# isri-aist/NMPC

Hardware: AMD Instinct MI355X
Metric: DDP iterations/s (whole node), batch=4096, T=100 (higher is better)
Workload: dtype f64

## Files before the change

### include/nmpc_amd/hip/ddp_kernels_quad.hpp

```cpp
#pragma once

#include <type_traits>

#include <nmpc_amd/hip/ddp_kernels_2w.hpp>

namespace nmpc_amd
{
namespace hip
{
constexpr int kQuadInstances = 16;
constexpr int kQuadWaves = 4;

template<class Problem, bool kConstrained, bool kFanOut = kConstrained>
struct QuadSolver : PairSolver<Problem, kConstrained, true, (kConstrained || kFanOut) ? 4 : 1, true>
{
  using Pair = PairSolver<Problem, kConstrained, true, (kConstrained || kFanOut) ? 4 : 1, true>;
  using Base = typename Pair::Base;
  using Base::b;
  using Base::buf;
  using Base::cfg;
  using Base::current_t;
  using Base::dV0;
  using Base::dV1;
  using Base::k_rel_norm;
  using Base::lambda;
  using Base::lane;
  using Base::problem;
  using Base::sel;
  using Base::T;
  static constexpr int N = Base::N;
  static constexpr int M = Base::M;
  static constexpr int MM = Base::MM;
  static constexpr size_t LW = Base::LW;
  using typename Base::InputDimVector;
  using typename Base::InputInputDimMatrix;
  using typename Base::QPOut;
  using typename Base::StateDimVector;
  using typename Base::StateInputDimMatrix;
  using typename Base::StateStateDimMatrix;

  static constexpr bool kShape = (N >= 1 && N <= 4 && M == 1 && !Problem::kDynamicInput);

  static constexpr int oFx = 0;
  static constexpr int oLxx = 16;
  static constexpr int oFu = 32;
  static constexpr int oLxu = 36;
  static constexpr int oLx = 40;
  static constexpr int oLuu = 44;
  static constexpr int oLu = 45;
  static constexpr int oU = 46;
  static constexpr int oLoRel = 46;
  static constexpr int oUpRel = 48;
  static constexpr int oZero = 47;
  static constexpr int kRecQ = 49;
  static constexpr int kChunkSteps = 16;
  static constexpr int gK = 0;
  static constexpr int gKfb = 1;
  static constexpr int gLive = 5;
  static constexpr int gDummy = 6;
  static constexpr int kGainRec = 7;
  static constexpr int kInstPad = 8;
  static constexpr int kChunkDoubles = 64 * (kRecQ + kGainRec) + 4 * kInstPad;
  static constexpr int kMailIn = 4;
  static constexpr int kMailOut = 4;
  static constexpr int kMailDoubles = (kMailIn + kMailOut) * kQuadInstances;
  static constexpr int kLdsDoubles = Pair::kLdsDoubles + kMailDoubles + kQuadWaves * kChunkDoubles;
  static constexpr size_t kLdsBytes = static_cast<size_t>(kLdsDoubles) * sizeof(double);

  const Problem & lin_problem;
  const int wave;
  const int wl;
  const int row, blk, col;
  double * mail;
  double * chunk;

  NMPC_D QuadSolver(const Problem & p,
                    const Problem & p_lin,
                    const nmpc_hip_ddp_config & c,
                    const DeviceBuffers & bf,
                    int global_lane,
                    double * lds_base)
  : Pair(p, c, bf, global_lane, lds_base), lin_problem(p_lin), wave(threadIdx.x / 64), wl(threadIdx.x % 64), row(wl / 16), blk((wl / 4) % 4),
    col(wl % 4), mail(lds_base + Pair::kLdsDoubles),
    chunk(lds_base + Pair::kLdsDoubles + kMailDoubles + (threadIdx.x / 64) * kChunkDoubles)
  {
  }

  NMPC_D double & mailIn(int inst, int f) const
  {
    return mail[f * kQuadInstances + inst];
  }
  NMPC_D double & mailOut(int inst, int f) const
  {
    return mail[(kMailIn + f) * kQuadInstances + inst];
  }

  NMPC_D static double mma(double a, double b_, double c)
  {
    return __builtin_amdgcn_mfma_f64_4x4x4f64(a, b_, c, 0, 0, 0);
  }
  template<int kSrc>
  NMPC_D static double quadBroadcast(double v)
  {
    constexpr int ctrl = kSrc | (kSrc << 2) | (kSrc << 4) | (kSrc << 6);
    const int lo = __builtin_amdgcn_update_dpp(0, __double2loint(v), ctrl, 0xf, 0xf, true);
    const int hi = __builtin_amdgcn_update_dpp(0, __double2hiint(v), ctrl, 0xf, 0xf, true);
    return __hiloint2double(hi, lo);
  }
  NMPC_D static double pick(bool p, double v)
  {
    return p ? v : 0.0;
  }

  struct PointQ
  {
    double x[N], u;
    double lo, hi;
  };
  NMPC_D static void loadPointQ(int i, const double * px, const double * pu, PointQ & p)
  {
#pragma unroll
    for(int j = 0; j < N; j++)
    {
      p.x[j] = px[(static_cast<size_t>(i) * N + j) * LW];
    }
    p.u = pu[static_cast<size_t>(i) * LW];
  }
  template<bool kFull>
  NMPC_D static void put(double * at, double v)
  {
    if(kFull || !__builtin_constant_p(v))
    {
      *at = v;
    }
  }
  template<bool kFull>
  NMPC_D double lineariseStep(int i, double t0_l, const PointQ & p, double * rec) const
  {
    const double t = t0_l + i * lin_problem.dt();
    StateDimVector x;
    InputDimVector u;
    u.resize(M);
#pragma unroll
    for(int j = 0; j < N; j++)
    {
      x[j] = p.x[j];
    }
    u[0] = p.u;
    StateStateDimMatrix Fx, Lxx;
    StateInputDimMatrix Fu, Lxu;
    StateDimVector Lx;
    InputDimVector Lu;
    InputInputDimMatrix Luu;
    Fu.resize(N, M);
    Lxu.resize(N, M);
    Lu.resize(M);
    Luu.resize(M, M);
    lin_problem.calcStateEqDeriv(t, x, u, Fx, Fu);
    lin_problem.calcRunningCostDeriv(t, x, u, Lx, Lu, Lxx, Luu, Lxu);
#pragma unroll
    for(int r = 0; r < 4; r++)
    {
#pragma unroll
      for(int c = 0; c < 4; c++)
      {
        put<kFull>(rec + oFx + 4 * r + c, (r < N && c < N) ? Fx(r < N ? r : 0, c < N ? c : 0) : 0.0);
        put<kFull>(rec + oLxx + 4 * r + c, (r < N && c < N) ? Lxx(r < N ? r : 0, c < N ? c : 0) : 0.0);
      }
      put<kFull>(rec + oFu + r, (r < N) ? Fu(r < N ? r : 0, 0) : 0.0);
      put<kFull>(rec + oLxu + r, (r < N) ? Lxu(r < N ? r : 0, 0) : 0.0);
      put<kFull>(rec + oLx + r, (r < N) ? Lx[r < N ? r : 0] : 0.0);
    }
    put<kFull>(rec + oLuu, Luu(0, 0));
    put<kFull>(rec + oLu, Lu[0]);
    if constexpr(kConstrained)
    {
      rec[oLoRel] = p.lo - u[0];
      rec[oUpRel] = p.hi - u[0];
    }
    else
    {
      rec[oU] = u[0];
    }
    put<kFull>(rec + oZero, 0.0);
    return recipFast(fabs(u[0]) + 1.0);
  }

  NMPC_D void backwardQuad() const
  {
    const int inst = wave * 4 + blk;
    const bool need = mailIn(inst, 0) != 0.0;
    const double lam = mailIn(inst, 1);
    const int lane_q = static_cast<int>(lane - lane % kQuadInstances) + inst;
    const int inst_l = wave * 4 + wl / 16;
    const int ts_l = wl % 16;
    const int sel_l = static_cast<int>(mailIn(inst_l, 2));
    const double t0_l = mailIn(inst_l, 3);
    const int lane_l = static_cast<int>(lane - lane % kQuadInstances) + inst_l;
    const double * px = Base::Xt + static_cast<size_t>(sel_l) * (Base::rowsX() * LW) + lane_l;
    const double * pu = Base::Ut + static_cast<size_t>(sel_l) * (Base::rowsU() * LW) + lane_l;
    double * rec_l = chunk + static_cast<size_t>(wl) * kRecQ + (wl / 16) * kInstPad;
    double * gains = chunk + 64 * kRecQ + 4 * kInstPad;
    const double * gain_l = gains + static_cast<size_t>(wl) * kGainRec;
    double * gain_q = gains + static_cast<size_t>(blk * 16) * kGainRec
                      + (row == 0 ? gKfb + col : ((row == 1 && col == 0) ? gK : ((row == 1 && col == 1) ? gLive : gDummy)));
    double * gain_u = gains + static_cast<size_t>(blk * 16) * kGainRec
                      + (row == 0 ? gKfb + col : ((row == 1 && col == 0) ? gK : gDummy));
    double * live_q = gains + static_cast<size_t>(blk * 16 + 4 * row + col) * kGainRec + gLive;
    const double * rec_q = chunk + static_cast<size_t>(blk * 16) * kRecQ + blk * kInstPad;

    const bool c0 = col == 0, c1 = col == 1, r0 = row == 0;
    const int aE = 4 * row + col;
    const int aT = 4 * col + row;
    const int aFuM = c0 ? oFu + row : oZero;
    const int aFuB = oFu + row;
    const int aLM = c0 ? oLxu + row : (c1 ? oLx + row : oZero);
    const int aCM = c0 ? oLuu : (c1 ? oLu : oZero);
    const int aLxuRow = oLxu + col;
    struct Operands
    {
      double Fx, Lxx, LxxT, FuM, FuB, LM, CM, LxuRow, lo, up;
    };
    auto loadOperands = [&](int ts, Operands & o)
    {
      const double * R = rec_q + static_cast<size_t>(ts) * kRecQ;
      o.Fx = R[oFx + aE];
      o.Lxx = R[oLxx + aE];
      o.LxxT = R[oLxx + aT];
      o.FuM = R[aFuM];
      o.FuB = R[aFuB];
      o.LM = R[aLM];
      o.CM = R[aCM];
      o.LxuRow = R[aLxuRow];
      if constexpr(kConstrained)
      {
        o.lo = R[oLoRel];
        o.up = R[oUpRel];
      }
    };

    if(ts_l == 0)
    {
      StateDimVector xT, vx;
      StateStateDimMatrix vxx;
#pragma unroll
      for(int j = 0; j < N; j++)
      {
        xT[j] = px[(static_cast<size_t>(T) * N + j) * LW];
      }
      lin_problem.calcTerminalCostDeriv(t0_l + T * lin_problem.dt(), xT, vx, vxx);
#pragma unroll
      for(int r = 0; r < 4; r++)
      {
#pragma unroll
        for(int c = 0; c < 4; c++)
        {
          rec_l[4 * r + c] = (r < N && c < N) ? vxx(r < N ? r : 0, c < N ? c : 0) : 0.0;
        }
        rec_l[16 + r] = (r < N) ? vx[r < N ? r : 0] : 0.0;
      }
    }
    double Vxx = rec_q[aE];
    double VxM = pick(c1, rec_q[16 + row]);

    double dV0_l = 0, dV1_l = 0;
    bool ok = true;
    double k_next = 0;
    bool have_next = false;
    const size_t tile_T = static_cast<size_t>(T);
    const int b_q = b - static_cast<int>(lane) + lane_q;

    auto step = [&](auto reg_tag, auto guarded_tag, int i, int ts, const Operands & o, int ts_next, Operands & o_next)
    {
      constexpr int kReg = decltype(reg_tag)::value;
      constexpr bool kGuarded = decltype(guarded_tag)::value;
      loadOperands(ts_next, o_next);
      const double P = mma(Vxx, o.Fx, 0.0);
      const double Rm = mma(Vxx, o.FuM, VxM);
      const double Qxx = mma(P, o.Fx, o.Lxx);
      const double QxxT = mma(o.Fx, P, o.LxxT);
      const double S = mma(o.Fx, Rm, o.LM);
      const double Wq = mma(o.FuB, Rm, o.CM);
      const double QA = mma(quadBroadcast<0>(Rm), o.Fx, o.LxuRow);
      const double Quu = quadBroadcast<0>(Wq);
      const double Qu = quadBroadcast<1>(Wq);
      const double Qr = quadBroadcast<0>(S);
      const double Qxr = quadBroadcast<1>(S);

      double Quu_F = Quu, QAr = QA, Qrr = Qr;
      if constexpr(kReg == 2)
      {
        const double VxxReg = (row == col) ? Vxx + lam : Vxx;
        const double R2 = mma(VxxReg, o.FuM, 0.0);
        Quu_F = quadBroadcast<0>(mma(o.FuB, R2, o.CM));
        QAr = mma(quadBroadcast<0>(R2), o.Fx, o.LxuRow);
        Qrr = quadBroadcast<0>(mma(o.Fx, R2, o.LM));
      }
      else if constexpr(kReg == 1)
      {
        Quu_F = Quu + lam;
      }

      double k, inv;
      bool step_ok;
      [[maybe_unused]] double qp_code = 0;
      if constexpr(kConstrained)
      {
        const double initial_k = (i != T - 1 && have_next) ? k_next : 0.0;
        QPOut qp;
#ifdef NMPC_AMD_PROFILE_QP
        asm volatile("s_nop 0" ::"v"(Quu_F), "v"(Qu));
        const unsigned long long tq = __builtin_readcyclecounter();
#endif
        Base::boxQP1Fast(Quu_F, Qu, o.lo, o.up, initial_k, qp);
#ifdef NMPC_AMD_PROFILE_QP
        asm volatile("s_nop 0" ::"v"(qp.x[0]), "v"(qp.retval));
        Pair::prof_wait += __builtin_readcyclecounter() - tq;
#endif
        qp_code = (need && ok) ? static_cast<double>(4 * (qp.retval + 8) + (qp.n_free > 0 ? 2 : 0)) : 0.0;
        step_ok = qp.retval >= 0;
        k = step_ok ? qp.x[0] : 0.0;
        inv = (step_ok && qp.n_free > 0) ? qp.inv_d[0] : 0.0;
      }
      else
      {
        step_ok = !(Quu_F <= 0);
        inv = (!kGuarded || step_ok) ? recipFast(Quu_F) : 0.0;
        k = -1 * (Qu * inv);
      }
      const double Kc = -1 * (QAr * inv);
      const double Kr = -1 * (Qrr * inv);
      const bool live = need && ok && step_ok;
      ok = ok && step_ok;

      if(!kGuarded || live)
      {
        dV0_l += k * Qu;
        dV1_l += 0.5 * (k * (Quu * k));
      }
      const double KQr = Kr * Quu, KQc = Kc * Quu;
      const double Vn = fma(Qr, Kc, fma(Kr, QA, fma(KQr, Kc, Qxx)));
      const double VnT = fma(QA, Kr, fma(Kc, Qr, fma(KQc, Kr, QxxT)));
      Vxx = 0.5 * (Vn + VnT);
      VxM = pick(c1, fma(Qr, k, fma(Kr, Qu, fma(KQr, k, Qxr))));

      if constexpr(kGuarded)
      {
        gain_q[static_cast<size_t>(ts) * kGainRec] = r0 ? Kc : (c0 ? k : (kConstrained ? qp_code + (live ? 1.0 : 0.0) : (live ? 1.0 : 0.0)));
      }
      else
      {
        gain_u[static_cast<size_t>(ts) * kGainRec] = r0 ? Kc : k;
      }
      k_next = k;
      have_next = true;
    };

    const int b_l = b - static_cast<int>(lane) + lane_l;
    auto loadLimits = [&](int i, PointQ & p)
    {
      if constexpr(kConstrained)
      {
        p.lo = inputLimitLo(buf, b_l, i, 0);
        p.hi = inputLimitHi(buf, b_l, i, 0);
      }
    };
    double krn_l = 0;
    auto flushGains = [&](int i_first, double uinv)
    {
      const int i = i_first + ts_l;
      const double flag = (i < T) ? gain_l[gLive] : 0.0;
      bool save = flag != 0.0;
      if constexpr(kConstrained)
      {
        const int code = static_cast<int>(flag);
        if(save)
        {
          Base::tileBase(buf.qp_ret, tile_T)[static_cast<size_t>(i) * LW + lane_l] = (code >> 2) - 8;
          Base::tileBase(buf.qp_free, tile_T)[static_cast<size_t>(i) * LW + lane_l] = static_cast<unsigned>((code >> 1) & 1);
        }
        save = (code & 1) != 0;
      }
      if(save)
      {
        const double kv = gain_l[gK];
        Base::kt[static_cast<size_t>(i) * LW + lane_l] = kv;
#pragma unroll
        for(int c = 0; c < N; c++)
        {
          Base::Kt[(static_cast<size_t>(i) * N + c) * LW + lane_l] = gain_l[gKfb + c];
        }
        krn_l = fmax(krn_l, fabs(kv) * uinv);
      }
    };
    auto runChunks = [&](auto reg_tag)
    {
      const int n_chunks = (T + kChunkSteps - 1) / kChunkSteps;
      PointQ pt;
      {
        const int i = ((n_chunks - 1) * kChunkSteps + ts_l < T) ? (n_chunks - 1) * kChunkSteps + ts_l : T - 1;
        loadPointQ(i, px, pu, pt);
        loadLimits(i, pt);
      }
      double uinv_prev = 0;
      for(int ch = n_chunks - 1; ch >= 0; ch--)
      {
        const int i0 = ch * kChunkSteps;
        double uinv_now;
        {
#ifdef NMPC_AMD_PROFILE_2W
          const unsigned long long tl = __builtin_readcyclecounter();
#endif
          const int i = (i0 + ts_l < T) ? i0 + ts_l : T - 1;
          uinv_now = (ch == n_chunks - 1) ? lineariseStep<true>(i, t0_l, pt, rec_l) : lineariseStep<false>(i, t0_l, pt, rec_l);
#ifdef NMPC_AMD_PROFILE_2W
          asm volatile("s_waitcnt lgkmcnt(0)" ::: "memory");
#ifndef NMPC_AMD_PROFILE_QP
          Pair::prof_wait += __builtin_readcyclecounter() - tl;
#endif
          Pair::prof_count++;
#endif
        }
        if(ch + 1 < n_chunks)
        {
          flushGains(i0 + kChunkSteps, uinv_prev);
        }
        uinv_prev = uinv_now;
        if(!Pair::kNominalTail || ch > 0)
        {
          const int in = i0 - kChunkSteps + ts_l;
          loadPointQ(in > 0 ? in : 0, px, pu, pt);
          loadLimits(in > 0 ? in : 0, pt);
        }
        const int hi = (i0 + kChunkSteps - 1 < T) ? i0 + kChunkSteps - 1 : T - 1;
#ifdef NMPC_AMD_QUAD_NO_STRAIGHT
        if constexpr(false)
#else
        if constexpr(!kConstrained)
#endif
        {
          const int n_steps = hi - i0 + 1;
          if((n_steps == kChunkSteps || n_steps == 4) && __all(ok))
          {
            const double Vxx_s = Vxx, VxM_s = VxM, dV0_s = dV0_l, dV1_s = dV1_l;
            auto straight = [&](auto r_tag)
            {
              constexpr int R = decltype(r_tag)::value;
              Operands o2[2];
              loadOperands(R - 1, o2[(R - 1) & 1]);
#pragma unroll
              for(int ts = R - 1; ts >= 0; ts--)
              {
                step(reg_tag, std::false_type(), i0 + ts, ts, o2[ts & 1], ts > 0 ? ts - 1 : 0, o2[(ts & 1) ^ 1]);
              }
            };
            if(n_steps == kChunkSteps)
            {
              straight(std::integral_constant<int, kChunkSteps>());
            }
            else
            {
              straight(std::integral_constant<int, 4>());
            }
            if(__all(ok))
            {
              *live_q = need ? 1.0 : 0.0;
              continue;
            }
            Vxx = Vxx_s;
            VxM = VxM_s;
            dV0_l = dV0_s;
            dV1_l = dV1_s;
            ok = true;
          }
        }
        Operands oa, ob;
        loadOperands(hi - i0, oa);
        int i = hi;
        for(; i - 1 >= i0; i -= 2)
        {
          step(reg_tag, std::true_type(), i, i - i0, oa, i - 1 - i0, ob);
          step(reg_tag, std::true_type(), i - 1, i - 1 - i0, ob, (i - 2 >= i0) ? i - 2 - i0 : 0, oa);
        }
        if(i >= i0)
        {
          step(reg_tag, std::true_type(), i, i - i0, oa, 0, ob);
        }
      }
      flushGains(0, uinv_prev);
      if constexpr(Pair::kNominalTail)
      {
        asm volatile("" ::: "memory");
        if(ts_l < 3 * Pair::kFwdGroup)
        {
          double * rec = Pair::nomRec(ts_l / Pair::kFwdGroup, ts_l % Pair::kFwdGroup, static_cast<unsigned>(inst_l));
#pragma unroll
          for(int j = 0; j < N; j++)
          {
            rec[j] = pt.x[j];
          }
          rec[N] = pt.u;
          rec[N + 1] = gain_l[gK];
#pragma unroll
          for(int c = 0; c < N; c++)
          {
            rec[N + 2 + c] = gain_l[gKfb + c];
          }
          if constexpr(Pair::kNomRec > N + 2 + N)
          {
            rec[Pair::kNomRec - 1] = 0;
          }
        }
      }
    };
    if(cfg.reg_type == 2)
    {
      runChunks(std::integral_constant<int, 2>());
    }
    else if(cfg.reg_type == 1)
    {
      runChunks(std::integral_constant<int, 1>());
    }
    else
    {
      runChunks(std::integral_constant<int, 0>());
    }
#pragma unroll
    for(int m = 8; m >= 1; m >>= 1)
    {
      krn_l = fmax(krn_l, __shfl_xor(krn_l, m, 16));
    }
    if(ts_l == 0)
    {
      mailOut(inst_l, 3) = krn_l;
    }
    if(r0 && c0)
    {
      mailOut(inst, 0) = ok ? 1.0 : 0.0;
      mailOut(inst, 1) = dV0_l;
      mailOut(inst, 2) = dV1_l;
    }
    fullBarrier();
  }

  NMPC_D bool backwardMasterQuad(bool need)
  {
    const int inst = wl % kQuadInstances;
    if(wl < kQuadInstances)
    {
      mailIn(inst, 0) = need ? 1.0 : 0.0;
      mailIn(inst, 1) = lambda;
      mailIn(inst, 2) = static_cast<double>(sel);
      mailIn(inst, 3) = current_t;
    }
    Pair::post(Pair::kCmdBackward);
    Pair::profBegin();
    backwardQuad();
    Pair::profEnd(0);
    const bool ok = mailOut(inst, 0) != 0.0;
    if(need)
    {
      dV0 = mailOut(inst, 1);
      dV1 = mailOut(inst, 2);
      k_rel_norm = mailOut(inst, 3);
    }
    return ok;
  }

  template<bool kResumable = false>
  NMPC_D void solveMasterQuad(bool valid)
  {
    if constexpr(kConstrained || kFanOut)
    {
      Pair::template solveMasterFanOut<kResumable>(valid, [this](bool need) { return backwardMasterQuad(need); });
    }
    else
    {
      Pair::template solveMasterWith<kResumable>(valid, [this](bool need) { return backwardMasterQuad(need); });
    }
  }

  NMPC_D void followerLoop() const
  {
    for(;;)
    {
      fullBarrier();
      const int word = static_cast<int>(Pair::mailFlags());
      const int cmd = __builtin_amdgcn_readfirstlane(word >> 1);
      const int sel_h = word & 1;
      if(cmd == Pair::kCmdExit)
      {
#ifdef NMPC_AMD_PROFILE_2W
        if(blockIdx.x == 0 && wl == 0)
        {
          buf.qp_free[static_cast<size_t>(4 + wave) * LW] = __builtin_amdgcn_s_getreg((15 << 11) | (0 << 6) | 4);
        }
#endif
        return;
      }
      if(cmd == Pair::kCmdBackward)
      {
        backwardQuad();
      }
      else if(cmd == Pair::kCmdAdoptFanOut)
      {
        Pair::adoptFanOut(sel_h);
      }
      else if(wave == 1)
      {
        if(cmd == Pair::kCmdForwardFanOut)
        {
          Pair::template forwardHelper<true>(sel_h);
        }
        else
        {
          Pair::forwardHelper(sel_h, cmd == Pair::kCmdRollout);
        }
      }
      else if(Pair::kExtraMasters > 0 && cmd == Pair::kCmdForwardFanOut && Pair::mailWidePass() != 0.0)
      {
        if(wave == 2)
        {
          Pair::template forwardCostOnlyLds<true>(sel_h, 0);
        }
        else
        {
          Pair::template forwardCostOnlyLds<false>(sel_h, 1);
        }
      }
      else if(Pair::kLdsNominalPath && (cmd == Pair::kCmdForward || cmd == Pair::kCmdForwardFanOut) && wave == 2)
      {
        Pair::forwardPrefetch(sel_h);
      }
      else
      {
        const int n_bar = T / Pair::kFwdGroup + 2
                          + ((Pair::kLdsNominalPath && (cmd == Pair::kCmdForward || cmd == Pair::kCmdForwardFanOut)) ? 1 : 0);
        for(int i = 0; i < n_bar; i++)
        {
          Pair::wgBarrier();
        }
      }
    }
  }

  static constexpr int kIngestRows = 32;
  static constexpr int kIngestLoads = kQuadInstances * kIngestRows / 64;
  static constexpr int kIngestPitch = kQuadInstances + 1;
  static_assert(kIngestRows * kIngestPitch <= kChunkDoubles, "the staging area is a wave's derivative chunk");
  using GlobalIn = const double __attribute__((address_space(1))) *;
  using GlobalOut = double __attribute__((address_space(1))) *;
  using LdsPtr = double __attribute__((address_space(3))) *;
  __device__ __attribute__((noinline)) static void ingestInputs(const double * in_t0,
                                                                const double * in_x0,
                                                                const double * in_u,
                                                                double * t0,
                                                                double * x0,
                                                                double * U,
                                                                int B,
                                                                int RU,
                                                                int b0,
                                                                double * stage_generic)
  {
    GlobalIn g_t0 = (GlobalIn)in_t0, g_x0 = (GlobalIn)in_x0, g_u = (GlobalIn)in_u;
    LdsPtr stage = (LdsPtr)stage_generic;
    const int wave_i = threadIdx.x / 64, l = threadIdx.x % 64;
    const size_t tile_i = static_cast<size_t>(b0) / LW;
    const int lane0 = b0 % static_cast<int>(LW);
    GlobalOut u_out = (GlobalOut)(U + tile_i * 2 * static_cast<size_t>(RU) * LW + lane0);
    for(int r0 = wave_i * kIngestRows; r0 < RU; r0 += kQuadWaves * kIngestRows)
    {
      double v[kIngestLoads];
      const int rr = l % kIngestRows, r = r0 + rr;
      NMPC_UNROLL
      for(int k = 0; k < kIngestLoads; k++)
      {
        const int bb = b0 + k * (64 / kIngestRows) + l / kIngestRows;
        const bool ok = bb < B && r < RU;
        v[k] = g_u[ok ? static_cast<size_t>(bb) * RU + r : 0];
        v[k] = ok ? v[k] : 0.0;
      }
      NMPC_UNROLL
      for(int k = 0; k < kIngestLoads; k++)
      {
        stage[rr * kIngestPitch + k * (64 / kIngestRows) + l / kIngestRows] = v[k];
      }
      asm volatile("" ::: "memory");
      NMPC_UNROLL
      for(int k = 0; k < kIngestLoads; k++)
      {
        const int rw = k * (64 / kQuadInstances) + l / kQuadInstances;
        v[k] = stage[rw * kIngestPitch + l % kQuadInstances];
      }
      NMPC_UNROLL
      for(int k = 0; k < kIngestLoads; k++)
      {
        const int rw = r0 + k * (64 / kQuadInstances) + l / kQuadInstances;
        if(rw < RU)
        {
          u_out[static_cast<size_t>(rw) * LW + l % kQuadInstances] = v[k];
        }
      }
      asm volatile("" ::: "memory");
    }
    if(wave_i == kQuadWaves - 1)
    {
      for(int e = l; e < kQuadInstances * N; e += 64)
      {
        const int inst = e / N, j = e % N;
        const bool ok = b0 + inst < B;
        const double xv = g_x0[ok ? static_cast<size_t>(b0) * N + e : 0];
        ((GlobalOut)x0)[tile_i * N * LW + static_cast<size_t>(j) * LW + lane0 + inst] = ok ? xv : 0.0;
      }
    }
    else if(wave_i == kQuadWaves - 2 && l < kQuadInstances)
    {
      const bool ok = in_t0 != nullptr && b0 + l < B;
      ((GlobalOut)t0)[tile_i * LW + lane0 + l] = ok ? g_t0[b0 + l] : 0.0;
    }
  }
};

template<class Problem, bool kConstrained, bool kOwnProblem = false, bool kFanOut = kConstrained, bool kResumable = false>
__global__ __launch_bounds__(kQuadWaves * 64) void ddp_solve_quad_kernel(const Problem problem,
                                                                         const nmpc_hip_ddp_config cfg,
                                                                         const DeviceBuffers buf)
{
  using Solver = QuadSolver<Problem, kConstrained, kFanOut>;
  extern __shared__ __attribute__((aligned(16))) double lds_quad[];
  const int wl = threadIdx.x % 64;
  int first = 0;
  bool solver_fresh = false;
  if constexpr(kResumable)
  {
    const int first_fresh = (buf.stream_mode != 0 && buf.first_active) ? *buf.first_active : 0;
    solver_fresh = buf.stream_mode == 2 && buf.first_active && static_cast<int>(blockIdx.x) * kQuadInstances >= first_fresh;
    first = (buf.stream_mode == 1) ? first_fresh : 0;
    if(static_cast<int>(blockIdx.x + 1) * kQuadInstances <= first
       || (buf.stream_mode != 0 && buf.n_active && static_cast<int>(blockIdx.x) * kQuadInstances >= *buf.n_active))
    {
      return;
    }
  }
  const int b = blockIdx.x * kQuadInstances + wl % kQuadInstances;
  const int b_lin = blockIdx.x * kQuadInstances + (threadIdx.x / 64) * 4 + wl / 16;
  const Problem mine = kOwnProblem ? instanceProblem(problem, buf, b) : problem;
  const Problem mine_lin = kOwnProblem ? instanceProblem(problem, buf, b_lin) : problem;
  Solver solver(mine, kOwnProblem ? mine_lin : mine, cfg, buf, b, lds_quad);
  solver.stream_fresh_wg = solver_fresh;
  if constexpr(!kResumable)
  {
    if(buf.in_x0 != nullptr)
    {
      Solver::ingestInputs(buf.in_t0, buf.in_x0, buf.in_u, const_cast<double *>(buf.t0), const_cast<double *>(buf.x0), buf.U, buf.B, buf.T * Solver::MM,
                           static_cast<int>(blockIdx.x) * kQuadInstances, solver.chunk);
      fullBarrier();
    }
  }
  if(threadIdx.x / 64 == 0)
  {
    if constexpr(kResumable)
    {
      solver.template solveMasterQuad<true>(b >= first && b < (buf.n_active ? *buf.n_active : buf.B));
    }
    else
    {
      solver.solveMasterQuad(b < buf.B);
    }
  }
  else
  {
    solver.current_t = buf.t0 ? solver.tileBase(buf.t0, 1)[solver.lane] : 0.0;
    solver.followerLoop();
  }
}
}
}
```

Baseline: 17410.

## Precompute constant record fields, use offset-based loads, defer Quu check in straight path

Writes the constant (zero) fields of each linearisation record once at kernel start, so every chunk uses the partial-write linearisation path. Replaces pointer arithmetic with 32-bit byte offsets that are decremented per chunk through Base::ld/st helpers. The unguarded straight-line path now tracks a running minimum of Quu with v_min_f64 and checks it once after the chunk instead of per step. Terminal value data moves into the gains area and the broadcast Qxr is replaced by S. The aim is fewer address calculations, fewer LDS stores and fewer per-step branches, at the cost of more complicated offset bookkeeping and possible overflow if the arrays grow large.

```diff
diff --git a/include/nmpc_amd/hip/ddp_kernels_quad.hpp b/include/nmpc_amd/hip/ddp_kernels_quad.hpp
--- a/include/nmpc_amd/hip/ddp_kernels_quad.hpp
+++ b/include/nmpc_amd/hip/ddp_kernels_quad.hpp
@@ -111,20 +111,26 @@
   {
     return p ? v : 0.0;
   }
+  NMPC_D static double minQuiet(double a, double b_)
+  {
+    double r;
+    asm("v_min_f64 %0, %1, %2" : "=v"(r) : "v"(a), "v"(b_));
+    return r;
+  }
 
   struct PointQ
   {
     double x[N], u;
     double lo, hi;
   };
-  NMPC_D static void loadPointQ(int i, const double * px, const double * pu, PointQ & p)
+  NMPC_D void loadPointQ(unsigned ox, unsigned ou, PointQ & p) const
   {
 #pragma unroll
     for(int j = 0; j < N; j++)
     {
-      p.x[j] = px[(static_cast<size_t>(i) * N + j) * LW];
-    }
-    p.u = pu[static_cast<size_t>(i) * LW];
+      p.x[j] = Base::ld(Base::Xt + j * LW, ox);
+    }
+    p.u = Base::ld(Base::Ut, ou);
   }
   template<bool kFull>
   NMPC_D static void put(double * at, double v)
@@ -185,6 +191,17 @@
     put<kFull>(rec + oZero, 0.0);
     return recipFast(fabs(u[0]) + 1.0);
   }
+  NMPC_D void layRecordConstants() const
+  {
+    PointQ p;
+#pragma unroll
+    for(int j = 0; j < N; j++)
+    {
+      p.x[j] = 0.0;
+    }
+    p.u = p.lo = p.hi = 0.0;
+    lineariseStep<true>(0, 0.0, p, chunk + static_cast<size_t>(wl) * kRecQ + (wl / 16) * kInstPad);
+  }
 
   NMPC_D void backwardQuad() const
   {
@@ -197,8 +214,10 @@
     const int sel_l = static_cast<int>(mailIn(inst_l, 2));
     const double t0_l = mailIn(inst_l, 3);
     const int lane_l = static_cast<int>(lane - lane % kQuadInstances) + inst_l;
-    const double * px = Base::Xt + static_cast<size_t>(sel_l) * (Base::rowsX() * LW) + lane_l;
-    const double * pu = Base::Ut + static_cast<size_t>(sel_l) * (Base::rowsU() * LW) + lane_l;
+    constexpr unsigned kRowB = static_cast<unsigned>(LW * sizeof(double));
+    const unsigned x_l = (static_cast<unsigned>(sel_l) * static_cast<unsigned>(Base::rowsX() * LW) + static_cast<unsigned>(lane_l)) * 8u;
+    const unsigned u_l = (static_cast<unsigned>(sel_l) * static_cast<unsigned>(Base::rowsU() * LW) + static_cast<unsigned>(lane_l)) * 8u;
+    const unsigned g_l = static_cast<unsigned>(lane_l) * 8u;
     double * rec_l = chunk + static_cast<size_t>(wl) * kRecQ + (wl / 16) * kInstPad;
     double * gains = chunk + 64 * kRecQ + 4 * kInstPad;
     const double * gain_l = gains + static_cast<size_t>(wl) * kGainRec;
@@ -246,25 +265,28 @@
 #pragma unroll
       for(int j = 0; j < N; j++)
       {
-        xT[j] = px[(static_cast<size_t>(T) * N + j) * LW];
+        xT[j] = Base::ld(Base::Xt + (static_cast<size_t>(T) * N + j) * LW, x_l);
       }
       lin_problem.calcTerminalCostDeriv(t0_l + T * lin_problem.dt(), xT, vx, vxx);
+      double * park_l = gains + static_cast<size_t>(wl) * kGainRec;
 #pragma unroll
       for(int r = 0; r < 4; r++)
       {
 #pragma unroll
         for(int c = 0; c < 4; c++)
         {
-          rec_l[4 * r + c] = (r < N && c < N) ? vxx(r < N ? r : 0, c < N ? c : 0) : 0.0;
-        }
-        rec_l[16 + r] = (r < N) ? vx[r < N ? r : 0] : 0.0;
-      }
-    }
-    double Vxx = rec_q[aE];
-    double VxM = pick(c1, rec_q[16 + row]);
+          park_l[4 * r + c] = (r < N && c < N) ? vxx(r < N ? r : 0, c < N ? c : 0) : 0.0;
+        }
+        park_l[16 + r] = (r < N) ? vx[r < N ? r : 0] : 0.0;
+      }
+    }
+    const double * park_q = gains + static_cast<size_t>(blk * 16) * kGainRec;
+    double Vxx = park_q[aE];
+    double VxM = pick(c1, park_q[16 + row]);
 
     double dV0_l = 0, dV1_l = 0;
     bool ok = true;
+    double quu_min = 0;
     double k_next = 0;
     bool have_next = false;
     const size_t tile_T = static_cast<size_t>(T);
@@ -285,7 +307,6 @@
       const double Quu = quadBroadcast<0>(Wq);
       const double Qu = quadBroadcast<1>(Wq);
       const double Qr = quadBroadcast<0>(S);
-      const double Qxr = quadBroadcast<1>(S);
 
       double Quu_F = Quu, QAr = QA, Qrr = Qr;
       if constexpr(kReg == 2)
@@ -324,7 +345,15 @@
       }
       else
       {
-        step_ok = !(Quu_F <= 0);
+        if constexpr(kGuarded)
+        {
+          step_ok = !(Quu_F <= 0);
+        }
+        else
+        {
+          quu_min = minQuiet(quu_min, Quu_F);
+          step_ok = true;
+        }
         inv = (!kGuarded || step_ok) ? recipFast(Quu_F) : 0.0;
         k = -1 * (Qu * inv);
       }
@@ -342,7 +371,7 @@
       const double Vn = fma(Qr, Kc, fma(Kr, QA, fma(KQr, Kc, Qxx)));
       const double VnT = fma(QA, Kr, fma(Kc, Qr, fma(KQc, Kr, QxxT)));
       Vxx = 0.5 * (Vn + VnT);
-      VxM = pick(c1, fma(Qr, k, fma(Kr, Qu, fma(KQr, k, Qxr))));
+      VxM = pick(c1, fma(Qr, k, fma(Kr, Qu, fma(KQr, k, S))));
 
       if constexpr(kGuarded)
       {
@@ -366,42 +395,46 @@
       }
     };
     double krn_l = 0;
-    auto flushGains = [&](int i_first, double uinv)
-    {
-      const int i = i_first + ts_l;
-      const double flag = (i < T) ? gain_l[gLive] : 0.0;
+    const int n_chunks = (T + kChunkSteps - 1) / kChunkSteps;
+    const int i_tail = (n_chunks - 1) * kChunkSteps + ts_l;
+    const bool tail_in_T = i_tail < T;
+    unsigned ox = x_l + static_cast<unsigned>(i_tail) * (N * kRowB), ou = u_l + static_cast<unsigned>(i_tail) * kRowB;
+    unsigned ok_g = g_l + static_cast<unsigned>(i_tail) * kRowB, oK_g = g_l + static_cast<unsigned>(i_tail) * (N * kRowB);
+    auto flushGains = [&](bool tail, double uinv)
+    {
+      const double flag = (tail && !tail_in_T) ? 0.0 : gain_l[gLive];
       bool save = flag != 0.0;
       if constexpr(kConstrained)
       {
         const int code = static_cast<int>(flag);
         if(save)
         {
-          Base::tileBase(buf.qp_ret, tile_T)[static_cast<size_t>(i) * LW + lane_l] = (code >> 2) - 8;
-          Base::tileBase(buf.qp_free, tile_T)[static_cast<size_t>(i) * LW + lane_l] = static_cast<unsigned>((code >> 1) & 1);
+          *reinterpret_cast<int *>(reinterpret_cast<char *>(Base::tileBase(buf.qp_ret, tile_T)) + (ok_g >> 1)) = (code >> 2) - 8;
+          *reinterpret_cast<unsigned *>(reinterpret_cast<char *>(Base::tileBase(buf.qp_free, tile_T)) + (ok_g >> 1)) =
+              static_cast<unsigned>((code >> 1) & 1);
         }
         save = (code & 1) != 0;
       }
       if(save)
       {
         const double kv = gain_l[gK];
-        Base::kt[static_cast<size_t>(i) * LW + lane_l] = kv;
+        Base::st(Base::kt, ok_g, kv);
 #pragma unroll
         for(int c = 0; c < N; c++)
         {
-          Base::Kt[(static_cast<size_t>(i) * N + c) * LW + lane_l] = gain_l[gKfb + c];
+          Base::st(Base::Kt + c * LW, oK_g, gain_l[gKfb + c]);
         }
         krn_l = fmax(krn_l, fabs(kv) * uinv);
       }
+      ok_g -= kChunkSteps * kRowB;
+      oK_g -= kChunkSteps * N * kRowB;
     };
     auto runChunks = [&](auto reg_tag)
     {
-      const int n_chunks = (T + kChunkSteps - 1) / kChunkSteps;
       PointQ pt;
-      {
-        const int i = ((n_chunks - 1) * kChunkSteps + ts_l < T) ? (n_chunks - 1) * kChunkSteps + ts_l : T - 1;
-        loadPointQ(i, px, pu, pt);
-        loadLimits(i, pt);
-      }
+      int i_pt = tail_in_T ? i_tail : T - 1;
+      loadPointQ(x_l + static_cast<unsigned>(i_pt) * (N * kRowB), u_l + static_cast<unsigned>(i_pt) * kRowB, pt);
+      loadLimits(i_pt, pt);
       double uinv_prev = 0;
       for(int ch = n_chunks - 1; ch >= 0; ch--)
       {
@@ -411,8 +444,8 @@
 #ifdef NMPC_AMD_PROFILE_2W
           const unsigned long long tl = __builtin_readcyclecounter();
 #endif
-          const int i = (i0 + ts_l < T) ? i0 + ts_l : T - 1;
-          uinv_now = (ch == n_chunks - 1) ? lineariseStep<true>(i, t0_l, pt, rec_l) : lineariseStep<false>(i, t0_l, pt, rec_l);
+          const int i = i_pt;
+          uinv_now = lineariseStep<false>(i, t0_l, pt, rec_l);
 #ifdef NMPC_AMD_PROFILE_2W
           asm volatile("s_waitcnt lgkmcnt(0)" ::: "memory");
 #ifndef NMPC_AMD_PROFILE_QP
@@ -423,14 +456,16 @@
         }
         if(ch + 1 < n_chunks)
         {
-          flushGains(i0 + kChunkSteps, uinv_prev);
+          flushGains(ch + 2 == n_chunks, uinv_prev);
         }
         uinv_prev = uinv_now;
-        if(!Pair::kNominalTail || ch > 0)
-        {
-          const int in = i0 - kChunkSteps + ts_l;
-          loadPointQ(in > 0 ? in : 0, px, pu, pt);
-          loadLimits(in > 0 ? in : 0, pt);
+        if(ch > 0)
+        {
+          ox -= kChunkSteps * N * kRowB;
+          ou -= kChunkSteps * kRowB;
+          i_pt = i0 - kChunkSteps + ts_l;
+          loadPointQ(ox, ou, pt);
+          loadLimits(i_pt, pt);
         }
         const int hi = (i0 + kChunkSteps - 1 < T) ? i0 + kChunkSteps - 1 : T - 1;
 #ifdef NMPC_AMD_QUAD_NO_STRAIGHT
@@ -443,6 +478,7 @@
           if((n_steps == kChunkSteps || n_steps == 4) && __all(ok))
           {
             const double Vxx_s = Vxx, VxM_s = VxM, dV0_s = dV0_l, dV1_s = dV1_l;
+            quu_min = __builtin_inf();
             auto straight = [&](auto r_tag)
             {
               constexpr int R = decltype(r_tag)::value;
@@ -462,7 +498,7 @@
             {
               straight(std::integral_constant<int, 4>());
             }
-            if(__all(ok))
+            if(__all(!(quu_min <= 0)))
             {
               *live_q = need ? 1.0 : 0.0;
               continue;
@@ -487,7 +523,7 @@
           step(reg_tag, std::true_type(), i, i - i0, oa, 0, ob);
         }
       }
-      flushGains(0, uinv_prev);
+      flushGains(n_chunks == 1, uinv_prev);
       if constexpr(Pair::kNominalTail)
       {
         asm volatile("" ::: "memory");
@@ -757,6 +793,7 @@
       fullBarrier();
     }
   }
+  solver.layRecordConstants();
   if(threadIdx.x / 64 == 0)
   {
     if constexpr(kResumable)
```

Result: faster. 18000 (median of 6 runs) (+3.4%).
